# neuzxy/Distributed-TF-Serving

Hardware: AMD Instinct MI355X
Metric: CTR scores/sec (whole node) (higher is better)
Workload: dtype bf16; 1 GPU; model=deepfm (1Mx64 emb, 43 fields, MLP 1024-512-256), global_batch=16384, request_rows=512, parallelism=candidate-dp1 (one GPU, no fan-out), encoding=raw, aux_lane_cus=0

## Files before the change

csrc/bindings_hip.cpp:

```cpp
#include <torch/extension.h>

#include <cstring>

#include <ATen/hip/HIPContext.h>
#include <c10/core/DeviceGuard.h>
#include <c10/hip/HIPStream.h>

#include "kernels/launchers.h"
#include "comm/rccl_comm.h"
#include "live_bindings.h"
#include "runtime/numa.h"
#include "runtime/step_runner.h"

namespace {

hipStream_t cur_stream(const torch::Tensor& t) { return c10::hip::getCurrentHIPStream(t.device().index()).stream(); }

void check_hip(hipError_t e, const char* what) {
  TORCH_CHECK(e == hipSuccess, what, " failed: ", hipGetErrorString(e));
}

void check_dev(const torch::Tensor& t, const char* name) {
  TORCH_CHECK(t.is_cuda(), name, " must be a GPU tensor");
  TORCH_CHECK(t.is_contiguous(), name, " must be contiguous");
// ... 1593 lines not shown
    TORCH_CHECK(S >= 1 && int(S) <= runner_->slots(), "slot count must be in [1, runner slots]");
    for (const auto& v : slots_) TORCH_CHECK(v.size() == S, "every bucket needs the same number of slots");
    auto add = [&](dtfs::comm::RcclComm* c) {
      if (c && std::find(comms_.begin(), comms_.end(), c) == comms_.end()) comms_.push_back(c);
    };
    for (const auto& v : slots_)
      for (const auto& s : v) {
        if (s.fanout)
          for (auto* c : {s.fan.cin, s.fan.cout}) add(c);
        if (s.program)
          for (const auto& o : s.prog.ops) add(o.comm);
      }
  }
  int slots() const override { return int(slots_[0].size()); }
  const std::vector<int64_t>& buckets() const override { return buckets_; }
  void set_scatter(dtfs::runtime::SharedScatter* sc, std::vector<int64_t> share_rows, int64_t timeout_us) {
    TORCH_CHECK(share_rows.size() == buckets_.size(), "shared scatter: one share row count per bucket");
    TORCH_CHECK(slots() <= dtfs::runtime::kScatterMaxSlots && slots() <= sc->slots(), "shared scatter: too many slots");
    sc_ = sc;
    share_rows_ = std::move(share_rows);
    slot_step_.assign(size_t(slots()), 0);
    timeout_us_ = timeout_us;
  }
  void launch(int slot, int b, const uint8_t* arena, const dtfs::runtime::ArenaBatch& batch) override {
    const auto& s = slots_[size_t(b)][size_t(slot)];
    if (sc_ && !s.program && !s.fanout) {
      slot_step_[size_t(slot)] = scatter_step(*runner_, *sc_, slot, share_rows_[size_t(b)], arena, s.h2d_dst,
                                              s.h2d_cap, s.seq, s.graph, timeout_us_);
      return;
    }
    const int64_t nbytes = batch.used_bytes;
    if (s.program) {
      if (nbytes > s.h2d_cap) throw std::runtime_error("batch larger than the device arena");
      runner_->launch_program(slot, s.prog, arena, nbytes, batch.n_gpu_varint == 0);
    } else if (s.fanout) {
      dtfs::runtime::FanoutStep f = s.fan;
      f.h2d_src = arena;
      f.h2d_bytes = nbytes;
      f.skip_varint = batch.n_gpu_varint == 0;
      runner_->launch_fanout(slot, f);
    } else {
      if (nbytes > s.h2d_cap) throw std::runtime_error("batch larger than the device arena");
      if (s.seq) runner_->launch_seq(slot, s.h2d_dst, arena, nbytes, s.seq, batch.n_gpu_varint == 0);
      else runner_->launch(slot, s.h2d_dst, arena, nbytes, s.graph);
    }
  }
  bool wait(int slot, int64_t timeout_us, std::string* err) override {
    if (sc_) return scatter_wait(*runner_, *sc_, slot, slot_step_[size_t(slot)], timeout_us, comms_, err);
    return runner_->wait_for(slot, timeout_us, comms_, err);
  }
  const float* scores(int slot, int b) const override { return slots_[size_t(b)][size_t(slot)].h_out; }
  int64_t scores_len(int slot, int b) const override { return slots_[size_t(b)][size_t(slot)].h_out_len; }
  const float* ranked_scores(int slot, int b) const override {
    return sc_ ? nullptr : slots_[size_t(b)][size_t(slot)].h_rank_val;
  }
  const int64_t* ranked_index(int slot, int b) const override {
    return sc_ ? nullptr : slots_[size_t(b)][size_t(slot)].h_rank_idx;
  }
  void abort() override {
    for (auto* c : comms_)
      if (c && !c->aborted()) c->abort();
  }

 private:
  dtfs::runtime::StepRunner* runner_;
  std::vector<int64_t> buckets_;
  std::vector<std::vector<dtfs::runtime::LoopSlot>> slots_;
  std::vector<dtfs::comm::RcclComm*> comms_;
  dtfs::runtime::SharedScatter* sc_ = nullptr;
  std::vector<int64_t> share_rows_;
  std::vector<uint64_t> slot_step_;
  int64_t timeout_us_ = 10'000'000;
};

struct PyGpuLive {
  std::vector<py::object> keep;
  std::unique_ptr<GpuBackend> backend;
  std::unique_ptr<dtfs::runtime::LiveServer> srv;
  ~PyGpuLive() {
    py::gil_scoped_release nogil;
    srv.reset();
  }
};

PyGpuLive* make_gpu_live(py::object runner_obj, py::dict cfg, py::list buckets, py::list arenas,
                         py::object control, py::object scatter, py::object share_rows) {
  auto* p = new PyGpuLive();
  dtfs::runtime::StepControl* ctl = dtfs_live::control_from(control, &p->keep);
  p->keep.push_back(runner_obj);
  auto& runner = runner_obj.cast<dtfs::runtime::StepRunner&>();
  std::vector<int64_t> rows;
  std::vector<std::vector<dtfs::runtime::LoopSlot>> slots;
  for (auto item : buckets) {
    py::tuple t = item.cast<py::tuple>();
    TORCH_CHECK(t.size() == 2, "bucket entries are (rows, slots)");
    rows.push_back(t[0].cast<int64_t>());
    std::vector<dtfs::runtime::LoopSlot> v;
    for (auto d : t[1].cast<py::list>()) v.push_back(loop_slot_from(d.cast<py::dict>(), &p->keep));
    slots.push_back(std::move(v));
  }
  auto ar = dtfs_live::arenas_from(arenas, true, &p->keep);
  p->backend = std::make_unique<GpuBackend>(&runner, std::move(rows), std::move(slots));
  if (auto* sc = dtfs_live::scatter_from(scatter, &p->keep)) {
    const auto lc = dtfs_live::live_config_from(cfg);
    p->backend->set_scatter(sc, share_rows.cast<std::vector<int64_t>>(), lc.step_timeout_us);
  }
  p->srv = std::make_unique<dtfs::runtime::LiveServer>(p->backend.get(), dtfs_live::live_config_from(cfg),
                                                       std::move(ar), ctl);
  return p;
}

}

PYBIND11_MODULE(_hip, m) {
  m.doc() = "distributed_tf_serving_amd gfx950 kernels (MFMA GEMM, embedding gather/bag, interactions, sort)";
  m.def("pack_ids", &pack_ids, py::arg("ids"), py::arg("modulo") = 0, py::arg("modulo_f") = py::none(),
        py::arg("offset_f") = py::none());
  m.def("embed", &embed, py::arg("table"), py::arg("lin"), py::arg("ids"), py::arg("wts"), py::arg("modulo"),
        py::arg("modulo_f") = py::none(), py::arg("offset_f") = py::none(), py::arg("bias") = 0.0,
        py::arg("want_x") = true, py::arg("want_fm") = false, py::arg("fm2") = false, py::arg("out_x") = py::none(),
        py::arg("validate_tables") = false, py::arg("shard_lo_f") = py::none(), py::arg("shard_n_f") = py::none(),
        py::arg("k_pad") = 0, py::arg("cross_w") = py::none(), py::arg("cross_c") = py::none());
  m.def("dense_pad", &dense_pad, py::arg("x"), py::arg("n"), py::arg("K"));
  m.def("embed_gemm", &embed_gemm, py::arg("table"), py::arg("lin"), py::arg("arena"), py::arg("ids"), py::arg("wts"),
        py::arg("B"), py::arg("F"), py::arg("modulo"), py::arg("bias"), py::arg("W"), py::arg("b"), py::arg("act"),
        py::arg("fm2"), py::arg("cross_w") = py::none(), py::arg("cross_c") = py::none(),
        py::arg("resolved") = py::none(), py::arg("Wp") = py::none());
  m.def("embed_gemm_resolve", &embed_gemm_resolve, py::arg("table"), py::arg("lin"), py::arg("arena"), py::arg("ids"),
        py::arg("wts"), py::arg("B"), py::arg("F"), py::arg("modulo"), py::arg("bias"), py::arg("n_parts"),
        "gather-GEMM front half (K1 resolve) -> (rows_t, wts_t, parts) for embed_gemm(resolved=...)");
  m.def("embed_arena", &embed_arena, py::arg("table"), py::arg("lin"), py::arg("arena"), py::arg("B"), py::arg("F"),
        py::arg("modulo"), py::arg("bias") = 0.0, py::arg("want_x") = true, py::arg("want_fm") = false,
        py::arg("fm2") = false, py::arg("out_x") = py::none(), py::arg("k_pad") = 0, py::arg("cross_w") = py::none(),
        py::arg("cross_c") = py::none());
  m.def("embedding_bag", &embedding_bag, py::arg("table"), py::arg("indices"), py::arg("offsets"),
        py::arg("per_sample_weights") = py::none(), py::arg("modulo") = 0, py::arg("mean") = false,
        py::arg("out_bf16") = false, py::arg("out") = py::none());
  m.def("gemm", &gemm, py::arg("A"), py::arg("W"), py::arg("bias") = py::none(), py::arg("epi") = 0,
        py::arg("x0") = py::none(), py::arg("xl") = py::none(), py::arg("out_f32") = false,
        py::arg("sa") = py::none(), py::arg("sw") = py::none(), py::arg("out") = py::none(),
        py::arg("variant") = 0, py::arg("sa_blk") = py::none(), py::arg("q_out") = py::none(),
        py::arg("sq_out") = py::none());
  m.def("cross_v1", &cross_v1, py::arg("x0"), py::arg("w"), py::arg("b"), py::arg("want_x") = true,
        py::arg("head_w") = py::none());
  m.def("dot_interaction", &dot_interaction, py::arg("dense"), py::arg("emb"), py::arg("out_cols") = 0,
        py::arg("emb_off") = py::none(), py::arg("emb_stride") = py::none());
  m.def("shard_route", &shard_route, py::arg("ids"), py::arg("arena"), py::arg("B"), py::arg("F"), py::arg("W"),
        py::arg("tm"), py::arg("col"), py::arg("mod"), py::arg("off"), py::arg("out") = py::none(),
        py::arg("hot") = 1, py::arg("wts") = py::none(), py::arg("out_w") = py::none(),
        "K1b routing: rows (+ weights) of every candidate's owned-table ids grouped by owner rank");
  m.def("dot_interaction_gather_peer", &dot_interaction_gather_peer, py::arg("dense"), py::arg("ids"),
        py::arg("arena"), py::arg("id_col0"), py::arg("cbase"), py::arg("towner"), py::arg("toff"), py::arg("trows"),
        py::arg("tremote"), py::arg("chunk_shift"), py::arg("cache") = py::none(), py::arg("stats") = py::none(),
        py::arg("ring") = py::none(), py::arg("ring_ctr") = py::none(), py::arg("sample_every") = 0,
        py::arg("out_cols") = 0,
        "K1 + K5 with the rows read where they live (peer stores over xGMI, replica cache first)");
  m.def("peer_bag", &peer_bag, py::arg("ids"), py::arg("wts"), py::arg("arena"), py::arg("B"), py::arg("col0"),
        py::arg("hot"), py::arg("cbase"), py::arg("towner"), py::arg("toff"), py::arg("trows"), py::arg("tremote"),
        py::arg("chunk_shift"), py::arg("cache") = py::none(), py::arg("stats") = py::none(),
        py::arg("ring") = py::none(), py::arg("ring_ctr") = py::none(), py::arg("sample_every") = 0, py::arg("out"),
        "K1b multi-hot bags with the rows read where they live -> bf16 [B, T, 64]");
  m.def("peer_cache_fill", &peer_cache_fill, py::arg("keys"), py::arg("slots"), py::arg("cbase"), py::arg("towner"),
        py::arg("toff"), py::arg("trows"), py::arg("tremote"), py::arg("chunk_shift"), py::arg("rows"),
        "replica cache: copy the keys' table rows into their slots");
  m.def("device_alloc", &device_alloc, py::arg("nbytes"), py::arg("like"),
        "uint8 device buffer of exactly nbytes (its own hipMalloc allocation)");
  m.def("cache_index_build", &cache_index_build, py::arg("keys"), py::arg("slots"), py::arg("entries"),
        "replica cache: open-addressing index keys -> slots ({key, slot} entries pre-filled with -1)");
  m.def("ipc_export", &ipc_export, py::arg("t"), "(IPC handle bytes, byte offset) of a device tensor's allocation");
  m.def("ipc_open", &ipc_open, py::arg("handle"), py::arg("offset"), py::arg("shape"), py::arg("like"),
        "map a peer's ipc_export as a tensor (dtype / device of `like`)");
  m.def("head", &head, py::arg("x"), py::arg("w"), py::arg("bias") = 0.0, py::arg("extra") = py::none(),
        py::arg("sigmoid") = true);
  m.def("gemm_head", &gemm_head, py::arg("A"), py::arg("W"), py::arg("bias"), py::arg("act"), py::arg("hw"),
        py::arg("hbias") = 0.0, py::arg("extra") = py::none(), py::arg("sigmoid") = true, py::arg("out") = py::none());
  m.def("mlp_tail", &mlp_tail, py::arg("X"), py::arg("W2p"), py::arg("b2"), py::arg("act2"), py::arg("W3p"),
        py::arg("b3"), py::arg("act3"), py::arg("hw"), py::arg("hbias") = 0.0, py::arg("extra") = py::none(),
        py::arg("sigmoid") = true, py::arg("out") = py::none());
  m.def("mlp_tail_fp8", &mlp_tail_fp8, py::arg("X"), py::arg("W2p"), py::arg("sw2"), py::arg("b2"), py::arg("act2"),
        py::arg("W3p"), py::arg("sw3"), py::arg("b3"), py::arg("act3"), py::arg("hw"), py::arg("hbias") = 0.0,
        py::arg("extra") = py::none(), py::arg("sigmoid") = true, py::arg("out") = py::none(),
        "MX-fp8 two-layer MLP tail + head in one launch, operands quantised in-kernel (mlp_tail_fp8.hip)");
  m.def("gather_mlp", &gather_mlp, py::arg("table"), py::arg("lin"), py::arg("arena"), py::arg("ids"),
        py::arg("wts"), py::arg("B"), py::arg("F"), py::arg("modulo"), py::arg("bias"), py::arg("W1p"), py::arg("b1"),
        py::arg("W2p"), py::arg("b2"), py::arg("act2"), py::arg("W3p"), py::arg("b3"), py::arg("act3"), py::arg("hw"),
        py::arg("hbias"), py::arg("fm"), py::arg("sigmoid") = true, py::arg("out") = py::none(),
        "DeepFM / Wide&Deep tower in one launch: resolve + gather + FM + 3 MLP layers + head (gather_mlp.hip)");
  m.def("set_embed_wave_cap", &dtfs::set_embed_wave_cap, py::arg("waves"), py::arg("rows_in_flight") = 1,
        "pipelined embedding gather geometry: resident-wave cap (0 = one row per wave) and rows in flight per "
        "wave (1 or 2); tuning sweeps and tests");
  m.def("quant_rows_fp8", &quant_rows_fp8, py::arg("x"), py::arg("k_pad") = 1);
  m.def("dot_interaction_gather", &dot_interaction_gather, py::arg("dense"), py::arg("table"), py::arg("ids"),
        py::arg("modulo_f"), py::arg("offset_f"), py::arg("out_cols") = 0);
  m.def("bottom_mlp3", &bottom_mlp3, py::arg("wts"), py::arg("nd"), py::arg("W1"), py::arg("b1"), py::arg("W2"),
        py::arg("b2"), py::arg("W3"), py::arg("b3"));
  m.def("bottom_mlp3_arena", &bottom_mlp3_arena, py::arg("arena"), py::arg("B"), py::arg("nd"), py::arg("W1"),
        py::arg("b1"), py::arg("W2"), py::arg("b2"), py::arg("W3"), py::arg("b3"));
  m.def("dot_interaction_gather_arena", &dot_interaction_gather_arena, py::arg("dense"), py::arg("table"),
        py::arg("arena"), py::arg("id_col0"), py::arg("modulo_f"), py::arg("offset_f"), py::arg("out_cols") = 0);
  m.def("cross_gemm_fp8", &cross_gemm_fp8, py::arg("q"), py::arg("sx"), py::arg("Wq"), py::arg("sw"), py::arg("bias"),
        py::arg("x0"), py::arg("xl"), py::arg("want_z") = true, py::arg("head_w") = py::none());
  m.def("cross_combine", &cross_combine, py::arg("y"), py::arg("x0"), py::arg("xl"), py::arg("want_z") = true,
        py::arg("k_pad") = 0, py::arg("head_w") = py::none(),
        "split DCN-v2 cross layer: z = x0*y + xl, optionally quantised (e4m3 + row scale) and/or dotted with head_w");
  m.def("unpack_arena", &unpack_arena, py::arg("arena"), py::arg("packed"), py::arg("fields"),
        py::arg("narrow_modulo") = 0);
  m.def("arena_varint_decode", &arena_varint_decode, py::arg("arena"), py::arg("blocks") = 256);
  m.def("pull_host", &pull_host, py::arg("dst"), py::arg("src"), py::arg("nbytes"), py::arg("blocks") = 128);
  m.def(
      "stream_write_u32",
      [](uintptr_t stream, torch::Tensor flag, uint32_t value) {
        TORCH_CHECK(flag.is_cuda() && flag.scalar_type() == torch::kInt32 && flag.numel() >= 1, "flag: int32 GPU tensor");
        check_hip(hipStreamWriteValue32(reinterpret_cast<hipStream_t>(stream), flag.data_ptr(), value, 0),
                  "hipStreamWriteValue32");
      },
      py::arg("stream"), py::arg("flag"), py::arg("value"));
  m.def(
      "stream_wait_u32",
      [](uintptr_t stream, torch::Tensor flag, uint32_t value) {
        TORCH_CHECK(flag.is_cuda() && flag.scalar_type() == torch::kInt32 && flag.numel() >= 1, "flag: int32 GPU tensor");
        check_hip(hipStreamWaitValue32(reinterpret_cast<hipStream_t>(stream), flag.data_ptr(), value,
                                       hipStreamWaitValueGte, 0xffffffffu),
                  "hipStreamWaitValue32");
      },
      py::arg("stream"), py::arg("flag"), py::arg("value"));
  m.def("sort_scores", &sort_scores, py::arg("scores"), py::arg("descending") = false, py::arg("k") = -1);
  m.def("rank_max_elems", &dtfs::rank_max_elems);
  m.def("rank_segments", &rank_segments, py::arg("scores"), py::arg("offsets"), py::arg("descending") = false,
        py::arg("k") = -1, py::arg("out_vals") = py::none(), py::arg("out_idx") = py::none());
  m.def("rank_arena", &rank_arena, py::arg("arena"), py::arg("scores"), py::arg("out_vals"), py::arg("out_idx"));
  m.def("sort_max_elems", &dtfs::sort_max_elems);

  py::class_<dtfs::runtime::StepRunner>(m, "StepRunner",
                                        "Native per-GPU step launcher: SDMA H2D + graph launch per pipeline slot")
      .def(py::init<int, int>(), py::arg("device"), py::arg("slots"))
      .def_property_readonly("aux_cus", &dtfs::runtime::StepRunner::aux_cus)
      .def(
          "launch",
          [](dtfs::runtime::StepRunner& r, int slot, torch::Tensor dst, torch::Tensor src, int64_t nbytes,
             uintptr_t graph_exec) {
            TORCH_CHECK(dst.is_cuda() && dst.is_contiguous(), "dst must be a contiguous GPU tensor");
            TORCH_CHECK(src.device().is_cpu() && src.is_contiguous() && src.is_pinned(),
                        "src must be a contiguous pinned host tensor");
            TORCH_CHECK(nbytes >= 0 && nbytes <= int64_t(dst.nbytes()) && nbytes <= int64_t(src.nbytes()),
                        "nbytes out of range");
            TORCH_CHECK(graph_exec != 0, "null graph exec");
            r.launch(slot, dst.data_ptr(), src.data_ptr(), nbytes, reinterpret_cast<hipGraphExec_t>(graph_exec));
          },
          py::arg("slot"), py::arg("dst"), py::arg("src"), py::arg("nbytes"), py::arg("graph_exec"))
      .def(
          "launch_fanout",
          [](dtfs::runtime::StepRunner& r, int slot, torch::Tensor h2d_dst, torch::Tensor h2d_src, int64_t h2d_bytes,
             uintptr_t ingress_exec, dtfs::comm::RcclComm& cin, int mode, torch::Tensor send, torch::Tensor recv,
             uintptr_t forward_exec, dtfs::comm::RcclComm& cout, torch::Tensor scores, torch::Tensor back,
             torch::Tensor h_out, int64_t d2h_bytes, uintptr_t resolve_exec) {
            TORCH_CHECK(h2d_src.device().is_cpu() && h2d_src.is_pinned(), "h2d_src must be pinned host memory");
            TORCH_CHECK(h2d_bytes >= 0 && h2d_bytes <= int64_t(h2d_dst.nbytes()) &&
                            h2d_bytes <= int64_t(h2d_src.nbytes()),
                        "h2d_bytes out of range");
            auto s = make_fanout_step(h2d_dst, ingress_exec, cin, mode, send, recv, forward_exec, cout, scores, back,
                                      h_out, d2h_bytes);
            s.h2d_src = h2d_src.data_ptr();
            s.h2d_bytes = h2d_bytes;
            s.resolve = reinterpret_cast<hipGraphExec_t>(resolve_exec);
            r.launch_fanout(slot, s);
          },
          py::arg("slot"), py::arg("h2d_dst"), py::arg("h2d_src"), py::arg("h2d_bytes"), py::arg("ingress_exec"),
          py::arg("cin"), py::arg("mode"), py::arg("send"), py::arg("recv"), py::arg("forward_exec"), py::arg("cout"),
          py::arg("scores"), py::arg("back"), py::arg("h_out"), py::arg("d2h_bytes"), py::arg("resolve_exec") = 0)
      .def(
          "launch_program",
          [](dtfs::runtime::StepRunner& r, int slot, py::dict program, torch::Tensor h2d_src, int64_t h2d_bytes) {
            std::vector<py::object> keep;
            auto p = program_from(program, &keep);
            torch::Tensor dst = program["h2d_dst"].cast<torch::Tensor>();
            TORCH_CHECK(h2d_src.device().is_cpu() && h2d_src.is_pinned(), "h2d_src must be pinned host memory");
            TORCH_CHECK(h2d_bytes >= 0 && h2d_bytes <= int64_t(dst.nbytes()) && h2d_bytes <= int64_t(h2d_src.nbytes()),
                        "h2d_bytes out of range");
            r.launch_program(slot, p, h2d_src.data_ptr(), h2d_bytes);
          },
          py::arg("slot"), py::arg("program"), py::arg("h2d_src"), py::arg("h2d_bytes"))
      .def("wait", &dtfs::runtime::StepRunner::wait, py::arg("slot"), py::call_guard<py::gil_scoped_release>())
      .def(
          "wait_for",
          [](dtfs::runtime::StepRunner& r, int slot, double timeout_s, std::vector<dtfs::comm::RcclComm*> comms) {
            std::string err;
            bool ok;
            {
              py::gil_scoped_release nogil;
              ok = r.wait_for(slot, int64_t(timeout_s * 1e6), comms, &err);
            }
            return py::make_tuple(ok, err);
          },
          py::arg("slot"), py::arg("timeout_s"), py::arg("comms") = std::vector<dtfs::comm::RcclComm*>(),
          "Bounded wait for the slot's step: (ok, error). Also polls the communicators' async errors.")
      .def("query", &dtfs::runtime::StepRunner::query, py::arg("slot"))
      .def_property_readonly("slots", &dtfs::runtime::StepRunner::slots)
      .def_property("feed_h2d", &dtfs::runtime::StepRunner::feed_h2d, &dtfs::runtime::StepRunner::set_feed_h2d,
                    "local steps: a feeder thread enqueues each step's kernels once the host sees its H2D landed "
                    "(True, default) instead of a device-side wait on the copy's event")
      .def_property("host_wait_h2d", &dtfs::runtime::StepRunner::host_wait_h2d,
                    &dtfs::runtime::StepRunner::set_host_wait_h2d,
                    "local steps: wait for each step's H2D on the host (True) or on the device (False)")
      .def_property_readonly("compute_stream",
                             [](const dtfs::runtime::StepRunner& r) { return reinterpret_cast<uintptr_t>(r.compute_stream()); });

  py::class_<dtfs::runtime::KernelSequence>(m, "KernelSequence",
                                            "A captured HIP graph replayed as direct kernel launches")
      .def(py::init([](uintptr_t graph) {
             TORCH_CHECK(graph != 0, "null hipGraph_t (capture with torch.cuda.CUDAGraph(keep_graph=True))");
             return std::make_unique<dtfs::runtime::KernelSequence>(reinterpret_cast<hipGraph_t>(graph));
           }),
           py::arg("graph"))
      .def(
          "launch",
          [](const dtfs::runtime::KernelSequence& s, uintptr_t stream) {
            s.launch(stream ? reinterpret_cast<hipStream_t>(stream)
                            : c10::hip::getCurrentHIPStream().stream());
          },
          py::arg("stream") = 0)
      .def_property_readonly("size", &dtfs::runtime::KernelSequence::size)
      .def("describe", &dtfs::runtime::KernelSequence::describe);

  {
    py::class_<PyGpuLive> c(m, "LiveServer",
                            "Live serving core (csrc/runtime/live_server.h) on this GPU: requests are batched into "
                            "pinned arenas and run as captured step kernels (or the fan-out step)");
    c.def(py::init(&make_gpu_live), py::arg("runner"), py::arg("config"), py::arg("buckets"), py::arg("arenas"),
          py::arg("control") = py::none(), py::arg("scatter") = py::none(), py::arg("share_rows") = py::none());
    dtfs_live::def_live_methods(c);
  }
  dtfs_live::def_step_control(m);
  dtfs_live::def_grpc_front<PyGpuLive>(m);
  {
    auto sc = dtfs_live::def_shared_scatter(m);
    sc.def(
          "register_with_gpu",
          [](dtfs::runtime::SharedScatter& s) {
            check_hip(hipHostRegister(s.base(), s.bytes(), hipHostRegisterMapped), "hipHostRegister(shared scatter)");
            s.set_on_unmap([](void* p, size_t) { (void)hipHostUnregister(p); });
          })
        .def(
            "launch",
            [](dtfs::runtime::SharedScatter& s, dtfs::runtime::StepRunner& r, int slot, int64_t rows_per_rank,
               c10::optional<torch::Tensor> arena, torch::Tensor dst, py::object seq, uintptr_t graph_exec,
               double timeout_s) {
              TORCH_CHECK(dst.is_cuda() && dst.is_contiguous() && dst.numel() >= s.arena_cap(),
                          "dst must be a device arena of the segment's capacity");
              const dtfs::runtime::KernelSequence* ks =
                  seq.is_none() ? nullptr : &seq.cast<dtfs::runtime::KernelSequence&>();
              TORCH_CHECK(ks || graph_exec, "need a kernel sequence or a graph");
              const uint8_t* a = arena ? static_cast<const uint8_t*>(arena->data_ptr()) : nullptr;
              return scatter_step(r, s, slot, rows_per_rank, a, dst.data_ptr(), int64_t(dst.nbytes()), ks,
                                  reinterpret_cast<hipGraphExec_t>(graph_exec), int64_t(timeout_s * 1e6));
            },
            py::arg("runner"), py::arg("slot"), py::arg("rows_per_rank"), py::arg("arena"), py::arg("dst"),
            py::arg("seq"), py::arg("graph_exec"), py::arg("timeout_s") = 10.0,
            "engine-level shared-scatter step (self-check); returns the step index")
        .def(
            "wait",
            [](dtfs::runtime::SharedScatter& s, dtfs::runtime::StepRunner& r, int slot, uint64_t k, double timeout_s) {
              std::string err;
              bool ok;
              {
                py::gil_scoped_release nogil;
                ok = scatter_wait(r, s, slot, k, int64_t(timeout_s * 1e6), {}, &err);
              }
              return py::make_tuple(ok, err);
            },
            py::arg("runner"), py::arg("slot"), py::arg("step"), py::arg("timeout_s") = 10.0);
  }

  m.def("rccl_set_library", &dtfs::comm::set_library, py::arg("path"));
  m.def(
      "alloc_pinned_on_node",
      [](int64_t bytes, int node) {
        void* p = dtfs::runtime::alloc_on_node(size_t(bytes), node);
        if (hipHostRegister(p, size_t(bytes), hipHostRegisterDefault) != hipSuccess) {
          dtfs::runtime::free_on_node(p, size_t(bytes));
          throw std::runtime_error("hipHostRegister failed");
        }
        const size_t n = size_t(bytes);
        return torch::from_blob(p, {bytes},
                                [n](void* q) {
                                  (void)hipHostUnregister(q);
                                  dtfs::runtime::free_on_node(q, n);
                                },
                                torch::TensorOptions().dtype(torch::kUInt8));
      },
      py::arg("bytes"), py::arg("node"));
  m.def(
      "pci_bus_id",
      [](int device) {
        char buf[64] = {0};
        if (hipDeviceGetPCIBusId(buf, sizeof(buf), device) != hipSuccess) return std::string();
        return std::string(buf);
      },
      py::arg("device"), "PCI bus id of a GPU (\"0000:65:00.0\"), for its NUMA node");
  m.def("rccl_unique_id", []() { return py::bytes(dtfs::comm::unique_id()); });
  py::class_<dtfs::comm::RcclComm>(m, "RcclComm", "Native RCCL communicator (fan-out collectives over xGMI)")
      .def(py::init([](py::bytes uid, int nranks, int rank, int device) {
             std::string id(uid);
             py::gil_scoped_release nogil;
             return std::make_unique<dtfs::comm::RcclComm>(id, nranks, rank, device);
           }),
           py::arg("uid"), py::arg("nranks"), py::arg("rank"), py::arg("device"))
      .def_property_readonly("rank", &dtfs::comm::RcclComm::rank)
      .def_property_readonly("nranks", &dtfs::comm::RcclComm::nranks)
      .def(
          "alltoall",
          [](dtfs::comm::RcclComm& c, torch::Tensor send, torch::Tensor recv) {
            TORCH_CHECK(send.is_cuda() && recv.is_cuda() && send.is_contiguous() && recv.is_contiguous(),
                        "contiguous GPU tensors");
            TORCH_CHECK(send.nbytes() == recv.nbytes() && send.nbytes() % c.nranks() == 0,
                        "send/recv must be equal and divisible by the world size");
            c10::DeviceGuard g(send.device());
            c.alltoall(send.data_ptr(), recv.data_ptr(), send.nbytes() / c.nranks(), cur_stream(send));
          },
          py::arg("send"), py::arg("recv"))
      .def(
          "allgather",
          [](dtfs::comm::RcclComm& c, torch::Tensor send, torch::Tensor recv) {
            TORCH_CHECK(send.is_cuda() && recv.is_cuda() && send.is_contiguous() && recv.is_contiguous(),
                        "contiguous GPU tensors");
            TORCH_CHECK(recv.nbytes() == send.nbytes() * c.nranks(), "recv must be world x send");
            c10::DeviceGuard g(send.device());
            c.allgather(send.data_ptr(), recv.data_ptr(), send.nbytes(), cur_stream(send));
          },
          py::arg("send"), py::arg("recv"))
      .def(
          "gather",
          [](dtfs::comm::RcclComm& c, torch::Tensor send, torch::Tensor recv, int root) {
            TORCH_CHECK(send.is_cuda() && recv.is_cuda() && send.is_contiguous() && recv.is_contiguous(),
                        "contiguous GPU tensors");
            TORCH_CHECK(root >= 0 && root < c.nranks(), "bad root");
            TORCH_CHECK(c.rank() != root || recv.nbytes() == send.nbytes() * c.nranks(), "root recv must be world x send");
            c10::DeviceGuard g(send.device());
            c.gather(send.data_ptr(), recv.data_ptr(), send.nbytes(), root, cur_stream(send));
          },
          py::arg("send"), py::arg("recv"), py::arg("root") = 0)
      .def(
          "scatter",
          [](dtfs::comm::RcclComm& c, torch::Tensor send, torch::Tensor recv, int root) {
            TORCH_CHECK(send.is_cuda() && recv.is_cuda() && send.is_contiguous() && recv.is_contiguous(),
                        "contiguous GPU tensors");
            TORCH_CHECK(root >= 0 && root < c.nranks(), "bad root");
            TORCH_CHECK(c.rank() != root || send.nbytes() == recv.nbytes() * c.nranks(), "root send must be world x recv");
            c10::DeviceGuard g(recv.device());
            c.scatter(send.data_ptr(), recv.data_ptr(), recv.nbytes(), root, cur_stream(recv));
          },
          py::arg("send"), py::arg("recv"), py::arg("root") = 0)
      .def(
          "peer_prepare", [](dtfs::comm::RcclComm& c, uint64_t cap) { return py::bytes(c.peer_prepare(cap)); },
          py::arg("cap"),
          "Allocate and export this rank's one-shot exchange mailbox (collective setup, step 1); returns its IPC handle")
      .def(
          "peer_enable",
          [](dtfs::comm::RcclComm& c, std::vector<py::bytes> handles, double timeout_s) {
            std::vector<std::string> h;
            for (auto& b : handles) h.emplace_back(std::string(b));
            c.peer_enable(h, timeout_s);
          },
          py::arg("handles"), py::arg("timeout_s") = 5.0,
          "Map every rank's mailbox (handles in rank order); messages <= cap then bypass RCCL")
      .def("can_access_device", &dtfs::comm::RcclComm::can_access_device, py::arg("device"),
           "hipDeviceCanAccessPeer from this communicator's device")
      .def_property_readonly("peer_enabled", &dtfs::comm::RcclComm::peer_enabled)
      .def_property_readonly("peer_cap", &dtfs::comm::RcclComm::peer_cap)
      .def_property_readonly("peer_exchanges", &dtfs::comm::RcclComm::peer_exchanges)
      .def("async_error", &dtfs::comm::RcclComm::async_error)
      .def("abort", &dtfs::comm::RcclComm::abort)
      .def_property_readonly("aborted", &dtfs::comm::RcclComm::aborted);
}
```

csrc/runtime/step_runner.cpp:

```cpp
#include "step_runner.h"

#include <algorithm>
#include <chrono>
#include <cstdio>
#include <cstdlib>
#include <cstring>
#include <stdexcept>
#include <string>
#include <thread>

namespace dtfs {
namespace runtime {

namespace {
void ck(hipError_t e, const char* what) {
  if (e != hipSuccess) throw std::runtime_error(std::string(what) + ": " + hipGetErrorString(e));
}
}

StepRunner::StepRunner(int device, int slots) : device_(device) {
  if (slots < 1) slots = 1;
  ck(hipSetDevice(device), "hipSetDevice");
  ck(hipStreamCreateWithFlags(&copy_, hipStreamNonBlocking), "hipStreamCreate(copy)");
  ck(hipStreamCreateWithFlags(&compute_, hipStreamNonBlocking), "hipStreamCreate(compute)");
  h2d_done_.resize(slots);
  done_.resize(slots);
  used_.assign(size_t(slots), 0);
  observed_.reset(new std::atomic<bool>[size_t(slots)]);
  for (int i = 0; i < slots; ++i) observed_[i].store(false);
  const unsigned done_flags = hipEventDisableTiming;
  for (int i = 0; i < slots; ++i) {
    ck(hipEventCreateWithFlags(&h2d_done_[i], hipEventDisableTiming), "hipEventCreate");
    ck(hipEventCreateWithFlags(&done_[i], done_flags), "hipEventCreate");
  }
  queued_.reset(new std::atomic<uint64_t>[size_t(slots)]);
  launched_.reset(new std::atomic<uint64_t>[size_t(slots)]);
  for (int i = 0; i < slots; ++i) {
    queued_[i].store(0);
    launched_[i].store(0);
  }
  if (const char* e = std::getenv("DTFS_FEED_H2D")) feed_h2d_ = std::atoi(e) != 0;
}

StepRunner::~StepRunner() {
  if (feeder_.joinable()) {
    {
      std::lock_guard<std::mutex> lk(feed_mu_);
      feed_stop_ = true;
    }
    feed_cv_.notify_all();
    feeder_.join();
  }
  hipSetDevice(device_);
  for (hipStream_t s : {compute_, copy_, copy2_, ingress_, egress_})
    if (s) hipStreamSynchronize(s);
  for (auto* v : {&h2d_done_, &done_, &in_done_, &fwd_done_, &prog_ev_})
    for (auto e : *v) hipEventDestroy(e);
  for (hipStream_t s : {compute_, copy_, copy2_, ingress_, egress_})
    if (s) hipStreamDestroy(s);
}

void StepRunner::ensure_aux_stream(bool program) {
  if (ingress_) return;
  int n = 0;
  if (program) {
    int cus = 0;
    (void)hipDeviceGetAttribute(&cus, hipDeviceAttributeMultiprocessorCount, device_);
    n = cus >= 256 ? cus / 2 : 0;
    if (const char* e = std::getenv("DTFS_AUX_CUS")) n = std::atoi(e);
    if (n >= cus) n = 0;
  }
  if (n > 0 && n < 256) {
    uint32_t mask[8] = {0, 0, 0, 0, 0, 0, 0, 0};
    for (int i = 0; i < n; ++i) mask[i / 32] |= 1u << (i % 32);
    ck(hipExtStreamCreateWithCUMask(&ingress_, 8, mask), "hipExtStreamCreateWithCUMask(ingress)");
    aux_cus_ = n;
    return;
  }
  ck(hipStreamCreateWithFlags(&ingress_, hipStreamNonBlocking), "hipStreamCreate(ingress)");
}

void StepRunner::ensure_fanout_streams() {
  if (egress_) return;
  ensure_aux_stream(false);
  ck(hipStreamCreateWithFlags(&egress_, hipStreamNonBlocking), "hipStreamCreate(egress)");
  in_done_.resize(done_.size());
  fwd_done_.resize(done_.size());
  for (size_t i = 0; i < done_.size(); ++i) {
    ck(hipEventCreateWithFlags(&in_done_[i], hipEventDisableTiming), "hipEventCreate");
    ck(hipEventCreateWithFlags(&fwd_done_[i], hipEventDisableTiming), "hipEventCreate");
  }
}

void StepRunner::copy_checked(void* dst, const void* src, int64_t nbytes, hipMemcpyKind kind, hipStream_t st,
                              int slot, const char* what) {
  const hipError_t e = hipMemcpyAsync(dst, src, size_t(nbytes), kind, st);
  if (e == hipSuccess) return;
  (void)hipGetLastError();
  auto describe = [](const void* p) {
    hipPointerAttribute_t at;
    std::memset(&at, 0, sizeof(at));
    const hipError_t q = hipPointerGetAttributes(&at, p);
    char buf[160];
    if (q != hipSuccess) {
      std::snprintf(buf, sizeof(buf), "%p (no HIP attributes: %s)", p, hipGetErrorString(q));
    } else {
      std::snprintf(buf, sizeof(buf), "%p (type %d, device %d, host %p, dev %p)", p, int(at.type), at.device,
                    at.hostPointer, at.devicePointer);
    }
    (void)hipGetLastError();
    return std::string(buf);
  };
  const std::string msg = std::string("hipMemcpyAsync(") + what + ", slot " + std::to_string(slot) + ", " +
                          std::to_string(nbytes) + " B): " + hipGetErrorString(e) + "; dst " + describe(dst) +
                          ", src " + describe(src);
  std::fprintf(stderr, "[step_runner] %s\n", msg.c_str());
  throw std::runtime_error(msg);
}

void StepRunner::h2d(int slot, void* dst, const void* src, int64_t nbytes, hipStream_t consumer, bool alternate) {
  std::vector<ShareCopy> one;
  if (nbytes > 0) one.push_back(ShareCopy{0, static_cast<const uint8_t*>(src), nbytes});
  h2d_copies(slot, dst, one, consumer, alternate);
}

void StepRunner::feed(const FeedJob& j) {
  if (!feeder_.joinable()) feeder_ = std::thread([this] { feeder_loop(); });
  queued_[j.slot].fetch_add(1, std::memory_order_acq_rel);
  {
    std::lock_guard<std::mutex> lk(feed_mu_);
    feed_q_.push_back(j);
  }
  feed_cv_.notify_one();
}

void StepRunner::feeder_loop() {
  try {
    ck(hipSetDevice(device_), "hipSetDevice(feeder)");
    for (;;) {
      FeedJob j;
      {
        std::unique_lock<std::mutex> lk(feed_mu_);
        feed_cv_.wait(lk, [&] { return feed_stop_ || !feed_q_.empty(); });
        if (feed_q_.empty()) return;
        j = feed_q_.front();
      }
      const auto t0 = std::chrono::steady_clock::now();
      for (;;) {
        const hipError_t e = hipEventQuery(h2d_done_[j.slot]);
        if (e == hipSuccess) break;
        if (e != hipErrorNotReady) ck(e, "hipEventQuery(h2d, feeder)");
        {
          std::lock_guard<std::mutex> lk(feed_mu_);
          if (feed_stop_) return;
        }
        if (std::chrono::steady_clock::now() - t0 < std::chrono::milliseconds(2)) std::this_thread::yield();
        else std::this_thread::sleep_for(std::chrono::microseconds(20));
      }
      if (j.program) {
        program_body(j.slot, j.prog, j.skip_varint, true);
      } else if (j.seq) {
        j.seq->launch(compute_, done_[j.slot], true, j.skip_varint);
      } else {
        ck(hipGraphLaunch(j.graph, compute_), "hipGraphLaunch(feeder)");
        ck(hipEventRecord(done_[j.slot], compute_), "hipEventRecord(done, feeder)");
      }
      {
        std::lock_guard<std::mutex> lk(feed_mu_);
        feed_q_.pop_front();
      }
      launched_[j.slot].fetch_add(1, std::memory_order_acq_rel);
    }
  } catch (const std::exception& e) {
    feed_error_ = e.what();
    feed_failed_.store(true, std::memory_order_release);
    std::fprintf(stderr, "[step_runner] feeder: %s\n", e.what());
  }
}

bool StepRunner::want_feed(int64_t nbytes) {
  if (!feed_h2d_ || host_wait_h2d_ || nbytes <= 0) return false;
  {
    std::lock_guard<std::mutex> lk(feed_mu_);
    if (!feed_q_.empty()) return true;
  }
  const int last = last_slot_;
  if (last < 0 || !slot_launched(last)) return last >= 0;
  return hipEventQuery(done_[last]) == hipErrorNotReady;
}

void StepRunner::wait_slot_launched(int slot) const {
  while (!slot_launched(slot) && !feed_failed_.load(std::memory_order_acquire)) std::this_thread::yield();
}

void StepRunner::drain_feeder() const {
  for (int s = 0; s < int(done_.size()); ++s) wait_slot_launched(s);
}

void StepRunner::h2d_copies(int slot, void* dst, const std::vector<ShareCopy>& copies, hipStream_t consumer,
                            bool alternate) {
  wait_slot_launched(slot);
  hipStream_t st = copy_;
  if (alternate) {
    if (!copy2_) ck(hipStreamCreateWithFlags(&copy2_, hipStreamNonBlocking), "hipStreamCreate(copy2)");
    if (n_h2d_++ & 1) st = copy2_;
  }
  if (used_[slot] && !observed_[slot].load(std::memory_order_acquire))
    ck(hipStreamWaitEvent(st, done_[slot], 0), "hipStreamWaitEvent(copy)");
  int64_t nbytes = 0;
  for (const ShareCopy& c : copies) {
    if (c.n <= 0) continue;
    copy_checked(static_cast<uint8_t*>(dst) + c.dst_off, c.src, c.n, hipMemcpyHostToDevice, st, slot, "H2D");
    nbytes += c.n;
  }
  ck(hipEventRecord(h2d_done_[slot], st), "hipEventRecord(h2d)");
  if (host_wait_h2d_ && consumer == compute_ && nbytes > 0) {
    for (;;) {
      const hipError_t e = hipEventQuery(h2d_done_[slot]);
      if (e == hipSuccess) break;
      if (e != hipErrorNotReady) ck(e, "hipEventQuery(h2d)");
      std::this_thread::yield();
    }
  } else if (consumer) {
    ck(hipStreamWaitEvent(consumer, h2d_done_[slot], 0), "hipStreamWaitEvent(h2d)");
  }
  observed_[slot].store(false, std::memory_order_release);
}

void StepRunner::launch_fanout(int slot, const FanoutStep& s) {
  if (slot < 0 || slot >= int(done_.size())) throw std::out_of_range("slot");
  if (!s.cin || !s.cout || !(s.forward || s.forward_seq))
    throw std::invalid_argument("fan-out step needs both communicators and a forward");
  ck(hipSetDevice(device_), "hipSetDevice");
  ensure_fanout_streams();
  drain_feeder();
  last_slot_ = slot;
  h2d(slot, s.h2d_dst, s.h2d_src, s.h2d_bytes, ingress_, false);
  fanout_body(slot, s);
  used_[slot] = 1;
}

void StepRunner::fanout_body(int slot, const FanoutStep& s) {
  hipStream_t in = ingress_;
  if (s.ingress_seq) s.ingress_seq->launch(in, nullptr, false, s.skip_varint);
  else if (s.ingress) ck(hipGraphLaunch(s.ingress, in), "hipGraphLaunch(ingress)");
  if (s.mode == 0) s.cin->alltoall(s.send, s.recv, s.in_bytes, in);
  else s.cin->scatter(s.send, s.recv, s.in_bytes, 0, in);
  if (s.resolve_seq) s.resolve_seq->launch(in);
  else if (s.resolve) ck(hipGraphLaunch(s.resolve, in), "hipGraphLaunch(resolve)");
  ck(hipEventRecord(in_done_[slot], in), "hipEventRecord(in)");
  ck(hipStreamWaitEvent(compute_, in_done_[slot], 0), "hipStreamWaitEvent(compute)");
  if (s.forward_seq) {
    s.forward_seq->launch(compute_, fwd_done_[slot]);
  } else {
    ck(hipGraphLaunch(s.forward, compute_), "hipGraphLaunch(forward)");
    ck(hipEventRecord(fwd_done_[slot], compute_), "hipEventRecord(fwd)");
  }
  ck(hipStreamWaitEvent(egress_, fwd_done_[slot], 0), "hipStreamWaitEvent(egress)");
  if (s.mode == 0) s.cout->alltoall(s.scores, s.back, s.out_bytes, egress_);
  else s.cout->gather(s.scores, s.back, s.out_bytes, 0, egress_);
  if (s.d2h_bytes > 0) copy_checked(s.h_out, s.back, s.d2h_bytes, hipMemcpyDeviceToHost, egress_, slot, "D2H");
  ck(hipEventRecord(done_[slot], egress_), "hipEventRecord(done)");
}

void StepProgram::validate() const {
  if (h2d_lane != 0 && h2d_lane != 1) throw std::invalid_argument("program: h2d_lane must be 0 or 1");
  int64_t aux_ops = h2d_lane == 1 ? 1 : 0, joined = 0;
  bool recorded[kProgEvents] = {};
  int64_t covers[kProgEvents] = {};
  for (const ProgOp& o : ops) {
    if (o.lane != 0 && o.lane != 1) throw std::invalid_argument("program: lane must be 0 or 1");
    switch (o.kind) {
      case ProgOp::kKernels:
        if (!o.seq && !o.graph) throw std::invalid_argument("program: kernels op without a sequence or graph");
        break;
      case ProgOp::kAllToAll:
      case ProgOp::kAllGather:
      case ProgOp::kReduceScatter:
        if (!o.comm || !o.send || !o.recv) throw std::invalid_argument("program: collective without buffers");
        break;
      case ProgOp::kRecord:
      case ProgOp::kWait:
      case ProgOp::kWaitPrev:
        if (o.event < 0 || o.event >= kProgEvents) throw std::invalid_argument("program: event index out of range");
        break;
      default:
        throw std::invalid_argument("program: bad op kind");
    }
    if (o.kind == ProgOp::kRecord) {
      recorded[o.event] = true;
      covers[o.event] = o.lane == 1 ? aux_ops : 0;
    } else if (o.kind == ProgOp::kWait) {
      if (!recorded[o.event]) throw std::invalid_argument("program: event waited before it is recorded");
      if (o.lane == 0) joined = std::max(joined, covers[o.event]);
    } else if (o.kind != ProgOp::kWaitPrev && o.lane == 1) {
      ++aux_ops;
    }
  }
  if (joined < aux_ops) throw std::invalid_argument("program: aux-lane work is not joined into the compute lane");
}


void StepRunner::launch_program(int slot, const StepProgram& p, const void* h2d_src, int64_t h2d_bytes,
                                bool skip_varint) {
  if (slot < 0 || slot >= int(done_.size())) throw std::out_of_range("slot");
  ck(hipSetDevice(device_), "hipSetDevice");
  const bool fed = want_feed(h2d_bytes);
  last_slot_ = slot;
  if (!fed) drain_feeder();
  ensure_aux_stream(true);
  if (prog_ev_.empty()) {
    prog_ev_.resize(done_.size() * kProgEvents);
    for (auto& e : prog_ev_)
      ck(hipEventCreateWithFlags(&e, hipEventDisableTiming | hipEventDisableSystemFence), "hipEventCreate(program)");
  }
  hipStream_t lanes[2] = {compute_, ingress_};
  if (fed) {
    h2d(slot, p.h2d_dst, h2d_src, h2d_bytes, nullptr, egress_ == nullptr);
    used_[slot] = 1;
    FeedJob j;
    j.slot = slot;
    j.skip_varint = skip_varint;
    j.program = true;
    j.prog = p;
    feed(j);
    return;
  }
  h2d(slot, p.h2d_dst, h2d_src, h2d_bytes, lanes[p.h2d_lane], egress_ == nullptr);
  program_body(slot, p, skip_varint, false);
  used_[slot] = 1;
}

void StepRunner::program_body(int slot, const StepProgram& p, bool skip_varint, bool fed) {
  hipStream_t lanes[2] = {compute_, ingress_};
  hipEvent_t* ev = &prog_ev_[size_t(slot) * kProgEvents];
  const ProgOp* last = p.ops.empty() ? nullptr : &p.ops.back();
  const bool bound = last && last->kind == ProgOp::kKernels && last->lane == 0 && last->seq;
  bool aux_work = false, trivial[kProgEvents] = {};
  for (const ProgOp& o : p.ops) {
    hipStream_t st = lanes[o.lane];
    if (fed) {
      const bool noop = o.kind == ProgOp::kKernels && o.seq && skip_varint && o.seq->empty_without_varint();
      if (o.lane == 1 && o.kind != ProgOp::kRecord && o.kind != ProgOp::kWait && o.kind != ProgOp::kWaitPrev && !noop)
        aux_work = true;
      if (o.kind == ProgOp::kRecord && o.lane == 1 && !aux_work) {
        trivial[o.event] = true;
        continue;
      }
      if (o.kind == ProgOp::kWait && trivial[o.event]) continue;
    }
    switch (o.kind) {
      case ProgOp::kKernels:
        if (o.seq) {
          if (bound && &o == last) o.seq->launch(st, done_[slot], true, skip_varint);
          else o.seq->launch(st, nullptr, false, skip_varint);
        } else {
          ck(hipGraphLaunch(o.graph, st), "hipGraphLaunch(program)");
        }
        break;
      case ProgOp::kAllToAll:
        o.comm->alltoall(o.send, o.recv, o.bytes, st);
        break;
      case ProgOp::kAllGather:
        o.comm->allgather(o.send, o.recv, o.bytes, st);
        break;
      case ProgOp::kReduceScatter:
        o.comm->reduce_scatter_bf16(o.send, o.recv, o.bytes, st);
        break;
      case ProgOp::kRecord:
        ck(hipEventRecord(ev[o.event], st), "hipEventRecord(program)");
        break;
      case ProgOp::kWait:
        ck(hipStreamWaitEvent(st, ev[o.event], 0), "hipStreamWaitEvent(program)");
        break;
      case ProgOp::kWaitPrev:
        if (last_prog_slot_ >= 0)
          ck(hipStreamWaitEvent(st, prog_ev_[size_t(last_prog_slot_) * kProgEvents + o.event], 0),
             "hipStreamWaitEvent(program prev)");
        break;
    }
  }
  if (!bound) ck(hipEventRecord(done_[slot], compute_), "hipEventRecord(done)");
  last_prog_slot_ = slot;
}

void StepRunner::launch(int slot, void* dst, const void* src, int64_t nbytes, hipGraphExec_t graph) {
  if (slot < 0 || slot >= int(done_.size())) throw std::out_of_range("slot");
  ck(hipSetDevice(device_), "hipSetDevice");
  drain_feeder();
  last_slot_ = slot;
  h2d(slot, dst, src, nbytes, compute_, true);
  ck(hipGraphLaunch(graph, compute_), "hipGraphLaunch");
  ck(hipEventRecord(done_[slot], compute_), "hipEventRecord(done)");
  used_[slot] = 1;
}

void StepRunner::launch_seq(int slot, void* dst, const void* src, int64_t nbytes, const KernelSequence* seq,
                            bool skip_varint) {
  if (slot < 0 || slot >= int(done_.size())) throw std::out_of_range("slot");
  if (!seq) throw std::invalid_argument("null kernel sequence");
  ck(hipSetDevice(device_), "hipSetDevice");
  const bool fed = want_feed(nbytes);
  last_slot_ = slot;
  if (fed) {
    h2d(slot, dst, src, nbytes, nullptr, true);
    used_[slot] = 1;
    feed(FeedJob{slot, seq, nullptr, skip_varint});
    return;
  }
  drain_feeder();
  h2d(slot, dst, src, nbytes, compute_, true);
  seq->launch(compute_, done_[slot], true, skip_varint);
  used_[slot] = 1;
}

void StepRunner::launch_copies(int slot, void* dst, const std::vector<ShareCopy>& copies, const KernelSequence* seq,
                               hipGraphExec_t graph, bool skip_varint) {
  if (slot < 0 || slot >= int(done_.size())) throw std::out_of_range("slot");
  if (!seq && !graph) throw std::invalid_argument("launch_copies: no kernel sequence or graph");
  ck(hipSetDevice(device_), "hipSetDevice");
  int64_t nbytes = 0;
  for (const ShareCopy& c : copies) nbytes += c.n > 0 ? c.n : 0;
  const bool fed = want_feed(nbytes);
  last_slot_ = slot;
  if (fed) {
    h2d_copies(slot, dst, copies, nullptr, true);
    used_[slot] = 1;
    feed(FeedJob{slot, seq, seq ? nullptr : graph, skip_varint});
    return;
  }
  drain_feeder();
  h2d_copies(slot, dst, copies, compute_, true);
  if (seq) {
    seq->launch(compute_, done_[slot], true, skip_varint);
  } else {
    ck(hipGraphLaunch(graph, compute_), "hipGraphLaunch");
    ck(hipEventRecord(done_[slot], compute_), "hipEventRecord(done)");
  }
  used_[slot] = 1;
}

void StepRunner::wait(int slot) {
  if (slot < 0 || slot >= int(done_.size())) throw std::out_of_range("slot");
  wait_slot_launched(slot);
  if (feed_failed_.load(std::memory_order_acquire)) throw std::runtime_error("step feeder: " + feed_error_);
  if (used_[slot]) ck(hipEventSynchronize(done_[slot]), "hipEventSynchronize");
  observed_[slot].store(true, std::memory_order_release);
}

bool StepRunner::wait_for(int slot, int64_t timeout_us, const std::vector<comm::RcclComm*>& comms,
                          std::string* err) {
  if (slot < 0 || slot >= int(done_.size())) throw std::out_of_range("slot");
  using clk = std::chrono::steady_clock;
  const auto t0 = clk::now();
  auto last_comm_check = t0;
  if (used_[slot]) {
    for (;;) {
      if (feed_failed_.load(std::memory_order_acquire)) {
        *err = "step feeder: " + feed_error_;
        return false;
      }
      const hipError_t e = slot_launched(slot) ? hipEventQuery(done_[slot]) : hipErrorNotReady;
      if (e == hipSuccess) break;
      if (e != hipErrorNotReady) {
        *err = std::string("hipEventQuery: ") + hipGetErrorString(e);
        return false;
      }
      const auto now = clk::now();
      const int64_t el = std::chrono::duration_cast<std::chrono::microseconds>(now - t0).count();
      if (el > timeout_us) {
        *err = "step not finished after " + std::to_string(el / 1000) + " ms";
        return false;
      }
      if (!comms.empty() && now - last_comm_check > std::chrono::milliseconds(1)) {
        last_comm_check = now;
        for (auto* c : comms) {
          if (!c) continue;
          std::string ce = c->async_error();
          if (!ce.empty()) {
            *err = "RCCL: " + ce;
            return false;
          }
        }
      }
      if (el < 2000) std::this_thread::yield();
      else std::this_thread::sleep_for(std::chrono::microseconds(50));
    }
  }
  for (auto* c : comms) {
    if (!c) continue;
    std::string ce = c->async_error();
    if (!ce.empty()) {
      *err = "RCCL: " + ce;
      return false;
    }
  }
  observed_[slot].store(true, std::memory_order_release);
  return true;
}

bool StepRunner::query(int slot) {
  if (!used_[slot]) return true;
  if (!slot_launched(slot)) {
    if (feed_failed_.load(std::memory_order_acquire)) throw std::runtime_error("step feeder: " + feed_error_);
    return false;
  }
  hipError_t e = hipEventQuery(done_[slot]);
  if (e == hipErrorNotReady) return false;
  ck(e, "hipEventQuery");
  observed_[slot].store(true, std::memory_order_release);
  return true;
}

}
}
```

csrc/runtime/step_runner.h:

```cpp
#pragma once

#include <hip/hip_runtime.h>

#include <atomic>
#include <condition_variable>
#include <cstdint>
#include <deque>
#include <memory>
#include <mutex>
#include <string>
#include <thread>
#include <vector>

#include "../comm/rccl_comm.h"
#include "kernel_seq.h"
#include "shared_scatter.h"

namespace dtfs {
namespace runtime {

struct FanoutStep {
  void* h2d_dst = nullptr;
  const void* h2d_src = nullptr;
  int64_t h2d_bytes = 0;
  hipGraphExec_t ingress = nullptr;
  comm::RcclComm* cin = nullptr;
  int mode = 0;
  const void* send = nullptr;
  void* recv = nullptr;
  size_t in_bytes = 0;
  hipGraphExec_t forward = nullptr;
  comm::RcclComm* cout = nullptr;
  const void* scores = nullptr;
  void* back = nullptr;
  size_t out_bytes = 0;
  void* h_out = nullptr;
  size_t d2h_bytes = 0;
  const KernelSequence* ingress_seq = nullptr;
  const KernelSequence* forward_seq = nullptr;
  hipGraphExec_t resolve = nullptr;
  const KernelSequence* resolve_seq = nullptr;
  bool skip_varint = false;
};

struct ProgOp {
  enum Kind : int {
    kKernels = 0,
    kAllToAll = 1,
    kAllGather = 2,
    kReduceScatter = 3,
    kRecord = 4,
    kWait = 5,
    kWaitPrev = 6,
  };
  int kind = kKernels;
  int lane = 0;
  int event = 0;
  const KernelSequence* seq = nullptr;
  hipGraphExec_t graph = nullptr;
  comm::RcclComm* comm = nullptr;
  const void* send = nullptr;
  void* recv = nullptr;
  size_t bytes = 0;
};
constexpr int kProgEvents = 8;

struct StepProgram {
  void* h2d_dst = nullptr;
  int h2d_lane = 1;
  std::vector<ProgOp> ops;
  void validate() const;
};

struct LoopSlot {
  void* h2d_dst = nullptr;
  int64_t h2d_cap = 0;
  hipGraphExec_t graph = nullptr;
  const KernelSequence* seq = nullptr;
  bool fanout = false;
  FanoutStep fan;
  bool program = false;
  StepProgram prog;
  const float* h_out = nullptr;
  int64_t h_out_len = 0;
  const float* h_rank_val = nullptr;
  const int64_t* h_rank_idx = nullptr;
};

class StepRunner {
 public:
  StepRunner(int device, int slots);
  ~StepRunner();
  StepRunner(const StepRunner&) = delete;
  StepRunner& operator=(const StepRunner&) = delete;

  void launch(int slot, void* dst, const void* src, int64_t nbytes, hipGraphExec_t graph);
  void launch_seq(int slot, void* dst, const void* src, int64_t nbytes, const KernelSequence* seq,
                  bool skip_varint = false);
  void launch_copies(int slot, void* dst, const std::vector<ShareCopy>& copies, const KernelSequence* seq,
                     hipGraphExec_t graph, bool skip_varint = false);
  void launch_fanout(int slot, const FanoutStep& s);
  void launch_program(int slot, const StepProgram& p, const void* h2d_src, int64_t h2d_bytes,
                      bool skip_varint = false);
  void wait(int slot);
  bool wait_for(int slot, int64_t timeout_us, const std::vector<comm::RcclComm*>& comms, std::string* err);
  bool query(int slot);
  int slots() const { return int(done_.size()); }
  int aux_cus() const { return aux_cus_; }
  hipStream_t compute_stream() const { return compute_; }
  hipStream_t copy_stream() const { return copy_; }
  void set_host_wait_h2d(bool v) { host_wait_h2d_ = v; }
  bool host_wait_h2d() const { return host_wait_h2d_; }
  void set_feed_h2d(bool v) { feed_h2d_ = v; }
  bool feed_h2d() const { return feed_h2d_; }

 private:
  int device_;
  void copy_checked(void* dst, const void* src, int64_t nbytes, hipMemcpyKind kind, hipStream_t st, int slot,
                    const char* what);
  void h2d(int slot, void* dst, const void* src, int64_t nbytes, hipStream_t consumer, bool alternate);
  void h2d_copies(int slot, void* dst, const std::vector<ShareCopy>& copies, hipStream_t consumer, bool alternate);
  hipStream_t copy2_ = nullptr;
  bool host_wait_h2d_ = false;
  uint64_t n_h2d_ = 0;
  std::unique_ptr<std::atomic<bool>[]> observed_;
  void ensure_fanout_streams();
  void ensure_aux_stream(bool program);
  hipStream_t copy_ = nullptr, compute_ = nullptr, ingress_ = nullptr, egress_ = nullptr;
  std::vector<hipEvent_t> h2d_done_, done_, in_done_, fwd_done_;
  std::vector<hipEvent_t> prog_ev_;
  int last_prog_slot_ = -1;
  int aux_cus_ = 0;
  std::vector<char> used_;

  struct FeedJob {
    int slot = 0;
    const KernelSequence* seq = nullptr;
    hipGraphExec_t graph = nullptr;
    bool skip_varint = false;
    bool program = false;
    StepProgram prog;
  };
  void program_body(int slot, const StepProgram& p, bool skip_varint, bool fed);
  void fanout_body(int slot, const FanoutStep& s);
  bool feed_h2d_ = true;
  std::thread feeder_;
  std::mutex feed_mu_;
  std::condition_variable feed_cv_;
  std::deque<FeedJob> feed_q_;
  bool feed_stop_ = false;
  std::atomic<bool> feed_failed_{false};
  std::string feed_error_;
  std::unique_ptr<std::atomic<uint64_t>[]> queued_, launched_;
  void feed(const FeedJob& j);
  void feeder_loop();
  bool slot_launched(int slot) const {
    return launched_[slot].load(std::memory_order_acquire) == queued_[slot].load(std::memory_order_acquire);
  }
  bool want_feed(int64_t nbytes);
  int last_slot_ = -1;
  void wait_slot_launched(int slot) const;
  void drain_feeder() const;
};

}
}
```

Measured before the change: 152.8 million scores/s.

## Alternate local steps across two compute streams to overlap consecutive steps

Adds a second compute stream and round-robins local step launches (graph, kernel sequence, copies) between the two streams, so one step's kernels can overlap with the next step's. It falls back to a single lane when aux/fan-out streams exist, when compute_stream is read by Python, or when DTFS_COMPUTE_LANES=1. The risks are contention between concurrent steps and hazards if slots share scratch buffers. Whether it runs depends on whether the harness reads compute_stream, which would pin the runner to one lane.

```diff
diff --git a/csrc/bindings_hip.cpp b/csrc/bindings_hip.cpp
--- a/csrc/bindings_hip.cpp
+++ b/csrc/bindings_hip.cpp
@@ -1919,8 +1919,14 @@
       .def_property("host_wait_h2d", &dtfs::runtime::StepRunner::host_wait_h2d,
                     &dtfs::runtime::StepRunner::set_host_wait_h2d,
                     "local steps: wait for each step's H2D on the host (True) or on the device (False)")
+      .def_property_readonly("compute_lanes", &dtfs::runtime::StepRunner::compute_lanes,
+                             "compute streams local steps alternate over: 2, or 1 (DTFS_COMPUTE_LANES=1, after the "
+                             "aux / fan-out streams were created, or after compute_stream was read)")
+      .def("ensure_fanout_streams", &dtfs::runtime::StepRunner::ensure_fanout_streams,
+           "create the fan-out streams now (the runner falls back to one compute lane)")
       .def_property_readonly("compute_stream",
-                             [](const dtfs::runtime::StepRunner& r) { return reinterpret_cast<uintptr_t>(r.compute_stream()); });
+                             [](dtfs::runtime::StepRunner& r) { return reinterpret_cast<uintptr_t>(r.compute_stream()); },
+                             "the step stream; reading it pins the runner to one compute lane");
 
   py::class_<dtfs::runtime::KernelSequence>(m, "KernelSequence",
                                             "A captured HIP graph replayed as direct kernel launches")
diff --git a/csrc/runtime/step_runner.cpp b/csrc/runtime/step_runner.cpp
--- a/csrc/runtime/step_runner.cpp
+++ b/csrc/runtime/step_runner.cpp
@@ -40,6 +40,23 @@
     launched_[i].store(0);
   }
   if (const char* e = std::getenv("DTFS_FEED_H2D")) feed_h2d_ = std::atoi(e) != 0;
+  if (const char* e = std::getenv("DTFS_COMPUTE_LANES")) lanes_ = std::atoi(e) >= 2 ? 2 : 1;
+}
+
+hipStream_t StepRunner::local_lane() {
+  if (compute_lanes() < 2) return compute_;
+  if (!compute2_) ck(hipStreamCreateWithFlags(&compute2_, hipStreamNonBlocking), "hipStreamCreate(compute2)");
+  return (n_local_++ & 1) ? compute2_ : compute_;
+}
+
+void StepRunner::single_lane() {
+  lanes_ = 1;
+  if (!compute2_) return;
+  drain_feeder();
+  ck(hipSetDevice(device_), "hipSetDevice");
+  ck(hipStreamSynchronize(compute2_), "hipStreamSynchronize(compute2)");
+  ck(hipStreamDestroy(compute2_), "hipStreamDestroy(compute2)");
+  compute2_ = nullptr;
 }
 
 StepRunner::~StepRunner() {
@@ -52,16 +69,17 @@
     feeder_.join();
   }
   hipSetDevice(device_);
-  for (hipStream_t s : {compute_, copy_, copy2_, ingress_, egress_})
+  for (hipStream_t s : {compute_, compute2_, copy_, copy2_, ingress_, egress_})
     if (s) hipStreamSynchronize(s);
   for (auto* v : {&h2d_done_, &done_, &in_done_, &fwd_done_, &prog_ev_})
     for (auto e : *v) hipEventDestroy(e);
-  for (hipStream_t s : {compute_, copy_, copy2_, ingress_, egress_})
+  for (hipStream_t s : {compute_, compute2_, copy_, copy2_, ingress_, egress_})
     if (s) hipStreamDestroy(s);
 }
 
 void StepRunner::ensure_aux_stream(bool program) {
   if (ingress_) return;
+  single_lane();
   int n = 0;
   if (program) {
     int cus = 0;
@@ -82,6 +100,7 @@
 
 void StepRunner::ensure_fanout_streams() {
   if (egress_) return;
+  ck(hipSetDevice(device_), "hipSetDevice");
   ensure_aux_stream(false);
   ck(hipStreamCreateWithFlags(&egress_, hipStreamNonBlocking), "hipStreamCreate(egress)");
   in_done_.resize(done_.size());
@@ -160,10 +179,10 @@
       if (j.program) {
         program_body(j.slot, j.prog, j.skip_varint, true);
       } else if (j.seq) {
-        j.seq->launch(compute_, done_[j.slot], true, j.skip_varint);
+        j.seq->launch(j.lane, done_[j.slot], true, j.skip_varint);
       } else {
-        ck(hipGraphLaunch(j.graph, compute_), "hipGraphLaunch(feeder)");
-        ck(hipEventRecord(done_[j.slot], compute_), "hipEventRecord(done, feeder)");
+        ck(hipGraphLaunch(j.graph, j.lane), "hipGraphLaunch(feeder)");
+        ck(hipEventRecord(done_[j.slot], j.lane), "hipEventRecord(done, feeder)");
       }
       {
         std::lock_guard<std::mutex> lk(feed_mu_);
@@ -214,7 +233,7 @@
     nbytes += c.n;
   }
   ck(hipEventRecord(h2d_done_[slot], st), "hipEventRecord(h2d)");
-  if (host_wait_h2d_ && consumer == compute_ && nbytes > 0) {
+  if (host_wait_h2d_ && consumer && (consumer == compute_ || consumer == compute2_) && nbytes > 0) {
     for (;;) {
       const hipError_t e = hipEventQuery(h2d_done_[slot]);
       if (e == hipSuccess) break;
@@ -389,9 +408,10 @@
   ck(hipSetDevice(device_), "hipSetDevice");
   drain_feeder();
   last_slot_ = slot;
-  h2d(slot, dst, src, nbytes, compute_, true);
-  ck(hipGraphLaunch(graph, compute_), "hipGraphLaunch");
-  ck(hipEventRecord(done_[slot], compute_), "hipEventRecord(done)");
+  hipStream_t lane = local_lane();
+  h2d(slot, dst, src, nbytes, lane, true);
+  ck(hipGraphLaunch(graph, lane), "hipGraphLaunch");
+  ck(hipEventRecord(done_[slot], lane), "hipEventRecord(done)");
   used_[slot] = 1;
 }
 
@@ -402,15 +422,21 @@
   ck(hipSetDevice(device_), "hipSetDevice");
   const bool fed = want_feed(nbytes);
   last_slot_ = slot;
+  hipStream_t lane = local_lane();
   if (fed) {
     h2d(slot, dst, src, nbytes, nullptr, true);
     used_[slot] = 1;
-    feed(FeedJob{slot, seq, nullptr, skip_varint});
+    FeedJob j;
+    j.slot = slot;
+    j.seq = seq;
+    j.skip_varint = skip_varint;
+    j.lane = lane;
+    feed(j);
     return;
   }
   drain_feeder();
-  h2d(slot, dst, src, nbytes, compute_, true);
-  seq->launch(compute_, done_[slot], true, skip_varint);
+  h2d(slot, dst, src, nbytes, lane, true);
+  seq->launch(lane, done_[slot], true, skip_varint);
   used_[slot] = 1;
 }
 
@@ -423,19 +449,26 @@
   for (const ShareCopy& c : copies) nbytes += c.n > 0 ? c.n : 0;
   const bool fed = want_feed(nbytes);
   last_slot_ = slot;
+  hipStream_t lane = local_lane();
   if (fed) {
     h2d_copies(slot, dst, copies, nullptr, true);
     used_[slot] = 1;
-    feed(FeedJob{slot, seq, seq ? nullptr : graph, skip_varint});
+    FeedJob j;
+    j.slot = slot;
+    j.seq = seq;
+    j.graph = seq ? nullptr : graph;
+    j.skip_varint = skip_varint;
+    j.lane = lane;
+    feed(j);
     return;
   }
   drain_feeder();
-  h2d_copies(slot, dst, copies, compute_, true);
+  h2d_copies(slot, dst, copies, lane, true);
   if (seq) {
-    seq->launch(compute_, done_[slot], true, skip_varint);
+    seq->launch(lane, done_[slot], true, skip_varint);
   } else {
-    ck(hipGraphLaunch(graph, compute_), "hipGraphLaunch");
-    ck(hipEventRecord(done_[slot], compute_), "hipEventRecord(done)");
+    ck(hipGraphLaunch(graph, lane), "hipGraphLaunch");
+    ck(hipEventRecord(done_[slot], lane), "hipEventRecord(done)");
   }
   used_[slot] = 1;
 }
diff --git a/csrc/runtime/step_runner.h b/csrc/runtime/step_runner.h
--- a/csrc/runtime/step_runner.h
+++ b/csrc/runtime/step_runner.h
@@ -107,7 +107,12 @@
   bool query(int slot);
   int slots() const { return int(done_.size()); }
   int aux_cus() const { return aux_cus_; }
-  hipStream_t compute_stream() const { return compute_; }
+  hipStream_t compute_stream() {
+    single_lane();
+    return compute_;
+  }
+  int compute_lanes() const { return lanes_ >= 2 && !ingress_ && !egress_ ? 2 : 1; }
+  void ensure_fanout_streams();
   hipStream_t copy_stream() const { return copy_; }
   void set_host_wait_h2d(bool v) { host_wait_h2d_ = v; }
   bool host_wait_h2d() const { return host_wait_h2d_; }
@@ -124,9 +129,13 @@
   bool host_wait_h2d_ = false;
   uint64_t n_h2d_ = 0;
   std::unique_ptr<std::atomic<bool>[]> observed_;
-  void ensure_fanout_streams();
   void ensure_aux_stream(bool program);
   hipStream_t copy_ = nullptr, compute_ = nullptr, ingress_ = nullptr, egress_ = nullptr;
+  hipStream_t compute2_ = nullptr;
+  int lanes_ = 2;
+  uint64_t n_local_ = 0;
+  hipStream_t local_lane();
+  void single_lane();
   std::vector<hipEvent_t> h2d_done_, done_, in_done_, fwd_done_;
   std::vector<hipEvent_t> prog_ev_;
   int last_prog_slot_ = -1;
@@ -140,6 +149,7 @@
     bool skip_varint = false;
     bool program = false;
     StepProgram prog;
+    hipStream_t lane = nullptr;
   };
   void program_body(int slot, const StepProgram& p, bool skip_varint, bool fed);
   void fanout_body(int slot, const FanoutStep& s);
```

Result: faster. 161.1 million scores/s (median of 6 runs) (+5.5%).
